# eezkni/UEGAN

Measured on AMD Instinct MI355X. Metric: train imgs/sec @512px bs=16 on 1/2/4/8 MI355X; infer ms/img, higher is better.
Workload: dtype bf16; 1 GPU; FiveK-shaped 512x512 batch=16/GPU, full G/D/VGG train step (trainer.py:77-119), conv_dim=32, seeded stand-in VGG19; global_batch=16, parallelism=dp1, pool_size=50, collective=none (1 rank), passes=batched (fused.py)

## Files before the change

include/uegan_hip.h:

```cpp
#ifndef UEGAN_HIP_H_
#define UEGAN_HIP_H_

#include <stddef.h>
#include <stdint.h>

#ifdef __cplusplus
extern "C" {
#endif

#define UEGAN_VERSION 105

enum { UEGAN_OK = 0, UEGAN_E_INVALID = -1, UEGAN_E_HIP = -2, UEGAN_E_UNSUPPORTED = -3 };
enum { UEGAN_F32 = 0, UEGAN_BF16 = 1 };
enum { UEGAN_PAD_ZERO = 0, UEGAN_PAD_REFLECT = 1 };
enum { UEGAN_ACT_NONE = 0, UEGAN_ACT_LRELU = 1, UEGAN_ACT_RELU = 2, UEGAN_ACT_TANH = 3,
       UEGAN_ACT_SIGMOID = 4,
       UEGAN_ACT_SWISH = 5, UEGAN_ACT_SELU = 6 };
enum { UEGAN_IMPL_AUTO = 0, UEGAN_IMPL_MFMA = 1, UEGAN_IMPL_DIRECT = 2, UEGAN_IMPL_MFMA_REGSTAGE = 3, UEGAN_IMPL_MFMA_GENERIC = 4 };

typedef void* uegan_stream_t;

int uegan_version(void);
const char* uegan_last_error(void);
int uegan_set_conv_impl(int impl);
enum {
  UEGAN_TUNE_SMALL_GRID = 0,
  UEGAN_TUNE_FOLD_MAX = 1,
  UEGAN_TUNE_HEADS_NO_CG = 2,
  UEGAN_TUNE_WIDE_MIN_GRID = 3,
  UEGAN_TUNE_TALL_MIN_GRID = 4,
  UEGAN_TUNE_TALL_RPW = 5,
  UEGAN_TUNE_TALL_REFLECT = 6,
  UEGAN_TUNE_FLAT_S2 = 7,
  UEGAN_TUNE_TOEP_HEADS = 8,
  UEGAN_TUNE_HEADS_MFMA = 9,
  UEGAN_TUNE_FWD_STATS = 10,
  UEGAN_TUNE_WGRAD_XCD = 11,
  UEGAN_TUNE_VGG_EPI = 12,
  UEGAN_TUNE_GAM_BWD = 13,
  UEGAN_TUNE_COUNT = 14
};
int uegan_set_tuning(int knob, int value, int* previous);
int uegan_selftest_mfma(void* scratch_4096_floats, uegan_stream_t stream);

typedef struct {
  char name[96];
  int64_t launches;
  double total_ms;
  double total_flops;
  double total_bytes;
} uegan_profile_entry;
int uegan_profile_begin(int max_records);
int uegan_profile_end(uegan_profile_entry* out, int max_entries, int* n_entries);

typedef struct {
  int32_t dtype;
  int32_t B, H, W;
  int32_t C1, C2;
  int32_t Ho, Wo, Cout;
  int32_t KH, KW, stride, pad;
  int32_t pad_mode;
  int32_t act;
  int32_t Cin_w, Cout_w;
// ... 181 lines not shown
int uegan_nima_dwconv3x3(const float* x_nhwc, const float* w_9c, const float* scale, const float* shift, float* y_nhwc, int B, int H, int W,
                         int C_pad, int stride, float lo, float hi, uegan_stream_t stream);
int uegan_nima_pwconv(const float* x_mk, const float* w_nk, const float* scale, const float* shift, const float* residual, float* y_mn,
                      int64_t M, int Cin_pad, int Cout_pad, float lo, float hi, uegan_stream_t stream);
int uegan_nima_head(const float* x_nhwc, const float* w, const float* bias, float* pooled, float* probs, float* mean, float* std, int B,
                    int HW, int C_pad, int C, int n_classes, uegan_stream_t stream);

int uegan_fill_zero(void* p, size_t bytes, uegan_stream_t stream);
int uegan_scalar_wsum(int n, const float* const* terms, const float* weights, float* total, float* scaled, uegan_stream_t stream);
int uegan_scalar_wsum_bwd(int n, const float* weights, const float* g, float* gout, uegan_stream_t stream);
int uegan_gather_scalars(int n, const float* const* src, float* out, uegan_stream_t stream);

size_t uegan_reduce_workspace_floats(int B, int HW, int C);
int uegan_instnorm_fwd(int dtype, const void* x, void* y, float* mean, float* rstd, float* tmp, int B, int HW, int C, float eps,
                       uegan_stream_t stream);
int uegan_instnorm_bwd(int dtype, const void* dy, const void* y, const float* rstd, void* dx, float* tmp, int B, int HW,
                       int C, uegan_stream_t stream);

size_t uegan_gam_bwd_ws_bytes(int dtype, int B, int HW, int C, int act);
int uegan_gam_bwd(int dtype, const void* g, const void* y, const void* x, const float* rstd, const void* w_ihwo, const void* add1,
                  const void* add2, int act, void* dz_enc, float* dw, int Cin_row, int Cin_w, int accumulate, void* workspace,
                  size_t workspace_bytes, int B, int HW, int C, uegan_stream_t stream);

int uegan_moments(int dtype, const void* x, float* mean, float* var, float* tmp, int B, int HW, int C, uegan_stream_t stream);
size_t uegan_moments_window_workspace_bytes(int B, int C);
int uegan_moments_window_acc(int dtype, const void* x, const void* x_lo, int B, int H, int W, int C, int y0, int y1, int x0, int x1, double* sum,
                             double* sumsq, void* tmp, uegan_stream_t stream);
int uegan_moments_finish(const double* sum, const double* sumsq, double count, float eps, float* mean, float* rstd, int n, uegan_stream_t stream);
int uegan_affine_act_fwd(int dtype, int act, const void* x, const float* scale, const float* shift, void* y, int B, int HW, int C,
                         uegan_stream_t stream);
int uegan_affine_act_bwd_sums(int dtype, int act, const void* gy, const void* x, const float* scale, const float* shift, float* sums,
                              float* tmp, int B, int HW, int C, uegan_stream_t stream);
int uegan_affine_act_bwd_apply(int dtype, int act, const void* gy, const void* x, const float* scale, const float* shift, const float* ca,
                               const float* cb, const float* cc, void* gx, int B, int HW, int C, uegan_stream_t stream);

size_t uegan_rahinge_workspace_floats(int nscales);
int uegan_rahinge_fwd(int nscales, const float* const* real, const float* const* fake, const int64_t* n,
                      int for_discriminator, float* loss, float* tmp, uegan_stream_t stream);
int uegan_rahinge_bwd(int nscales, const float* const* real, const float* const* fake, const int64_t* n,
                      int for_discriminator, const float* tmp, const float* gscale, float* const* greal,
                      float* const* gfake, uegan_stream_t stream);
size_t uegan_rahinge_heads_workspace_floats(int nscales);
int uegan_rahinge_heads_fwd(int dtype, int nscales, const void* const* maps, const int64_t* pix_per_image, int nb, int cp, int ngroups,
                            int npairs, const int32_t* pairs, int for_discriminator, float* loss, float* tmp, uegan_stream_t stream);
int uegan_rahinge_heads_bwd(int dtype, int nscales, const void* const* maps, const int64_t* pix_per_image, int nb, int cp, int ngroups,
                            int npairs, const int32_t* pairs, int for_discriminator, const float* tmp, const float* gscale,
// ... 83 lines not shown
```

uegan_amd/_lib.py:

```python
import ctypes as C
import os

_HERE = os.path.dirname(os.path.abspath(__file__))
LIB_PATH = os.path.join(_HERE, "libuegan_hip.so")
LIB_PATH_F16 = os.path.join(_HERE, "libuegan_hip_f16.so")

_lib = None
_lib_f16 = None
_use_f16 = False
_emulated = False

c_int, c_i64, c_f32, c_vp, c_sz = C.c_int, C.c_int64, C.c_float, C.c_void_p, C.c_size_t


class ConvDesc(C.Structure):
    _fields_ = [(n, C.c_int32) for n in ("dtype", "B", "H", "W", "C1", "C2", "Ho", "Wo", "Cout", "KH", "KW", "stride", "pad",
                                          "pad_mode", "act", "Cin_w", "Cout_w", "Cin_total", "scale_group")]


class ProfileEntry(C.Structure):
    _fields_ = [("name", C.c_char * 96), ("launches", c_i64), ("total_ms", C.c_double), ("total_flops", C.c_double),
                ("total_bytes", C.c_double)]


# ... 69 lines not shown
    "uegan_conv2d_wgrad_acc": (c_int, [C.POINTER(ConvDesc), c_vp, c_vp, c_vp, c_vp, c_vp, c_vp, c_vp, c_sz, c_int, c_vp]),
    "uegan_act_bwd": (c_int, [c_int, c_int, c_vp, c_vp, c_vp, c_i64, c_vp]),
    "uegan_act_bwd2": (c_int, [c_int, c_int, c_vp, c_vp, c_vp, c_vp, c_i64, c_vp]),
    "uegan_act_bwd3": (c_int, [c_int, c_int, c_vp, c_vp, c_vp, c_vp, c_vp, c_i64, c_vp]),
    "uegan_nchw_to_nhwc": (c_int, [c_int, c_vp, c_vp, c_int, c_int, c_int, c_int, c_int, C.POINTER(c_f32), C.POINTER(c_f32), c_vp]),
    "uegan_nhwc_to_nchw": (c_int, [c_int, c_vp, c_vp, c_int, c_int, c_int, c_int, c_int, C.POINTER(c_f32), c_vp]),
    "uegan_residual_clamp_fwd": (c_int, [c_int, c_vp, c_vp, c_vp, c_int, c_int, c_int, c_int, c_int, c_vp]),
    "uegan_residual_clamp_bwd": (c_int, [c_int, c_vp, c_vp, c_vp, c_vp, c_vp, c_int, c_int, c_int, c_int, c_int, c_vp]),
    "uegan_residual_clamp_bwd_act": (c_int, [c_int, c_int, c_vp, c_vp, c_vp, c_vp, c_vp, c_int, c_int, c_int, c_int, c_int, c_vp]),
    "uegan_mul_bwd_act": (c_int, [c_int, c_int, c_int, c_vp, c_vp, c_vp, c_vp, c_vp, c_i64, c_vp]),
    "uegan_mul_fwd": (c_int, [c_int, c_vp, c_vp, c_vp, c_i64, c_vp]),
    "uegan_mul_bwd": (c_int, [c_int, c_vp, c_vp, c_vp, c_vp, c_vp, c_i64, c_vp]),
    "uegan_upsample2x_fwd": (c_int, [c_int, c_vp, c_vp, c_int, c_int, c_int, c_int, c_vp]),
    "uegan_upsample2x_fwd_at": (c_int, [c_int, c_vp, c_vp, c_int, c_int, c_int, c_int, c_int, c_int, c_int, c_int, c_vp]),
    "uegan_upsample2x_bwd": (c_int, [c_int, c_vp, c_vp, c_int, c_int, c_int, c_int, c_vp]),
    "uegan_maxpool2x2_fwd": (c_int, [c_int, c_vp, c_vp, c_int, c_int, c_int, c_int, c_vp]),
    "uegan_maxpool2x2_bwd": (c_int, [c_int, c_vp, c_vp, c_vp, c_int, c_int, c_int, c_int, c_vp]),
    "uegan_maxpool2x2_bwd_act": (c_int, [c_int, c_int, c_vp, c_vp, c_vp, c_int, c_int, c_int, c_int, c_vp]),
    "uegan_reduce_workspace_floats": (c_sz, [c_int, c_int, c_int]),
    "uegan_instnorm_fwd": (c_int, [c_int, c_vp, c_vp, c_vp, c_vp, c_vp, c_int, c_int, c_int, c_f32, c_vp]),
    "uegan_instnorm_bwd": (c_int, [c_int, c_vp, c_vp, c_vp, c_vp, c_vp, c_int, c_int, c_int, c_vp]),
    "uegan_gam_bwd_ws_bytes": (c_sz, [c_int, c_int, c_int, c_int, c_int]),
    "uegan_gam_bwd": (c_int, [c_int, c_vp, c_vp, c_vp, c_vp, c_vp, c_vp, c_vp, c_int, c_vp, c_vp, c_int, c_int, c_int, c_vp, c_sz, c_int, c_int, c_int, c_vp]),
    "uegan_moments": (c_int, [c_int, c_vp, c_vp, c_vp, c_vp, c_int, c_int, c_int, c_vp]),
    "uegan_moments_window_workspace_bytes": (c_sz, [c_int, c_int]),
    "uegan_moments_window_acc": (c_int, [c_int, c_vp, c_vp, c_int, c_int, c_int, c_int, c_int, c_int, c_int, c_int, c_vp, c_vp, c_vp, c_vp]),
    "uegan_moments_finish": (c_int, [c_vp, c_vp, C.c_double, c_f32, c_vp, c_vp, c_int, c_vp]),
    "uegan_affine_act_fwd": (c_int, [c_int, c_int, c_vp, c_vp, c_vp, c_vp, c_int, c_int, c_int, c_vp]),
    "uegan_affine_act_bwd_sums": (c_int, [c_int, c_int, c_vp, c_vp, c_vp, c_vp, c_vp, c_vp, c_int, c_int, c_int, c_vp]),
    "uegan_affine_act_bwd_apply": (c_int, [c_int, c_int, c_vp, c_vp, c_vp, c_vp, c_vp, c_vp, c_vp, c_vp, c_int, c_int, c_int, c_vp]),
    "uegan_rals_fwd": (c_int, [c_int, C.POINTER(c_vp), C.POINTER(c_vp), C.POINTER(c_i64), c_int, c_vp, c_vp, c_vp]),
    "uegan_rals_bwd": (c_int, [c_int, C.POINTER(c_vp), C.POINTER(c_vp), C.POINTER(c_i64), c_int, c_vp, c_vp, C.POINTER(c_vp), C.POINTER(c_vp), c_vp]),
    "uegan_pred_loss_fwd": (c_int, [c_int, c_f32, c_int, C.POINTER(c_vp), C.POINTER(c_i64), c_vp, c_vp, c_vp]),
    "uegan_pred_loss_bwd": (c_int, [c_int, c_f32, c_int, C.POINTER(c_vp), C.POINTER(c_i64), c_vp, C.POINTER(c_vp), c_vp]),
    "uegan_rahinge_fwd": (c_int, [c_int, C.POINTER(c_vp), C.POINTER(c_vp), C.POINTER(c_i64), c_int, c_vp, c_vp, c_vp]),
    "uegan_rahinge_bwd": (c_int, [c_int, C.POINTER(c_vp), C.POINTER(c_vp), C.POINTER(c_i64), c_int, c_vp, c_vp, C.POINTER(c_vp),
                                  C.POINTER(c_vp), c_vp]),
    "uegan_rahinge_heads_workspace_floats": (c_sz, [c_int]),
    "uegan_rahinge_heads_fwd": (c_int, [c_int, c_int, C.POINTER(c_vp), C.POINTER(c_i64), c_int, c_int, c_int, c_int, C.POINTER(C.c_int32), c_int,
                                        c_vp, c_vp, c_vp]),
    "uegan_rahinge_heads_bwd": (c_int, [c_int, c_int, C.POINTER(c_vp), C.POINTER(c_i64), c_int, c_int, c_int, c_int, C.POINTER(C.c_int32), c_int,
                                        c_vp, c_vp, C.POINTER(c_vp), C.c_uint32, c_vp]),
    "uegan_msrec_scratch_floats": (c_sz, []),
    "uegan_msrec_fwd": (c_int, [c_vp, c_vp, c_vp, c_vp, c_int, c_int, c_int, c_int, c_int, c_int, c_vp]),
    "uegan_msrec_bwd": (c_int, [c_vp, c_vp, c_vp, c_vp, c_int, c_int, c_int, c_int, c_int, c_int, c_vp]),
    "uegan_msl1_scratch_floats": (c_sz, []),
# ... 135 lines not shown
```

uegan_amd/csrc/common.h:

```cpp
#pragma once
#include <hip/hip_runtime.h>
#include <stdint.h>
#include <stddef.h>

#include "../../include/uegan_hip.h"

#ifdef UEGAN_TOOLS_BUILD
#define UEGAN_ABL_BITS(x) (x)
#else
#define UEGAN_ABL_BITS(x) 0
#endif

namespace uegan {

extern int g_tuning[UEGAN_TUNE_COUNT];
extern int g_abl_stream, g_abl_wide;


typedef uint16_t bf16_t;

typedef float f32x4 __attribute__((ext_vector_type(4)));
typedef short s16x8 __attribute__((ext_vector_type(8)));
typedef uint32_t u32x4 __attribute__((ext_vector_type(4)));
typedef uint32_t u32x2 __attribute__((ext_vector_type(2)));
// ... 154 lines not shown
}

__device__ __forceinline__ void percep_scalars(float weight, const float* gscale, int B, int HW, int C, float& k, float& inv_n) {
  const float nel = (float)B * (float)HW * (float)C;
  k = 2.f * weight * (gscale ? *gscale : 1.f) / nel;
  inv_n = 1.f / (float)HW;
}
__device__ __forceinline__ void percep_consts(const float* st, const float* tot, size_t bc, size_t o, float k, float inv_n, float& mx, float& rx,
                                              float& my, float& ry, float& mg, float& mgx) {
  mx = st[o]; rx = st[bc + o]; my = st[2 * bc + o]; ry = st[3 * bc + o];
  mg = k * tot[o * 3 + 1] * inv_n;
  mgx = k * tot[o * 3 + 2] * inv_n;
}
__device__ __forceinline__ float percep_tap_grad(float x, float y, float mx, float rx, float my, float ry, float k, float mg, float mgx) {
  const float xh = (x - mx) * rx, yh = (y - my) * ry;
  return rx * (k * (xh - yh) - mg - xh * mgx);
}

__host__ __device__ __forceinline__ int reflect_idx(int i, int n) {
  i = i < 0 ? -i : i;
  return i >= n ? 2 * (n - 1) - i : i;
}

__device__ __forceinline__ float wave_sum(float v) {
#pragma unroll
  for (int o = 32; o > 0; o >>= 1) v += __shfl_xor(v, o, 64);
  return v;
}

__device__ __forceinline__ float block_sum(float v, float* red) {
  v = wave_sum(v);
  const int lane = threadIdx.x & 63, w = threadIdx.x >> 6;
  __syncthreads();
  if (lane == 0) red[w] = v;
  __syncthreads();
  const int nw = (blockDim.x + 63) >> 6;
  float s = 0.f;
  for (int i = 0; i < nw; ++i) s += red[i];
  return s;
}

template <int N>
__device__ __forceinline__ void wait_vmcnt() {
  __builtin_amdgcn_s_waitcnt((N & 15) | (7 << 4) | (15 << 8) | ((N >> 4) << 14));
}
__device__ __forceinline__ void raw_barrier() { __builtin_amdgcn_s_barrier(); }
// ... 22 lines not shown
```

uegan_amd/csrc/conv_internal.h:

```cpp
#pragma once
#include <hip/hip_runtime.h>

#include "../../include/uegan_hip.h"

namespace uegan {
bool heads_applicable(const uegan_conv_desc* d);
int heads_fwd(const uegan_conv_desc* d, const void* x, const void* w_ohwi, const float* bias, const float* scale, void* y, hipStream_t s);
bool heads_dgrad_applicable(const uegan_conv_desc* d);
int heads_dgrad(const uegan_conv_desc* d, const void* dz, const void* w_ihwo, const float* scale, void* dx, hipStream_t s);
int heads_wgrad_blocks(const uegan_conv_desc* d);
int heads_wgrad(const uegan_conv_desc* d, const void* x, const void* dz, float* ws, hipStream_t s);
void percep_tap_consts(int dtype, const float* tmp, int B, int HW, int C, const float** st, const float** tot);
int instnorm_bwd_sums(int dtype, const void* dy, const void* y, float* tmp, int B, int HW, int C, hipStream_t s, const float** tot);
int wgrad_reduce_1x1(const float* ws, float* dw, int nsplit, int N, int C, int Cin_w, int Cin_row, size_t pstride, int acc, hipStream_t s);
}
```

uegan_amd/csrc/elementwise.hip:

```cpp
#include "common.h"
#include "launch.h"

namespace uegan {

struct Affine4 {
  float a[4], b[4];
  int on;
};

template <typename T>
__global__ void nchw_to_nhwc_kernel(const float* x, T* y, int B, int C, int Cp, int HW, Affine4 af, int pair) {
  constexpr int EPC = DT<T>::EPC;
  const int nch = Cp / EPC;
  const size_t total = (size_t)B * HW * nch;
  for (size_t i = (size_t)blockIdx.x * blockDim.x + threadIdx.x; i < total; i += (size_t)gridDim.x * blockDim.x) {
    const int ch = (int)(i % nch);
    const size_t p = i / nch;
    const int b = (int)(p / HW);
    const size_t hw = p - (size_t)b * HW;
    float v[EPC];
#pragma unroll
    for (int e = 0; e < EPC; ++e) {
      const int c = ch * EPC + e;
      v[e] = 0.f;
// ... 67 lines not shown
    Vec<T, V>::ld(b + i, bv);
#pragma unroll
    for (int e = 0; e < V; ++e) av[e] *= bv[e];
    Vec<T, V>::st(y + i, av);
  }
}
template <typename T, int V>
__global__ void mul_bwd_kernel(const T* g, const T* a, const T* b, T* da, T* db, size_t n, int act_a, int act_b) {
  for (size_t i = ((size_t)blockIdx.x * blockDim.x + threadIdx.x) * V; i < n; i += (size_t)gridDim.x * blockDim.x * V) {
    float gv[V], av[V], bv[V];
    Vec<T, V>::ld(g + i, gv);
    Vec<T, V>::ld(a + i, av);
    Vec<T, V>::ld(b + i, bv);
#pragma unroll
    for (int e = 0; e < V; ++e) {
      const float t = gv[e];
      gv[e] = t * bv[e] * act_grad_from_out(av[e], act_a);
      bv[e] = t * av[e] * act_grad_from_out(bv[e], act_b);
    }
    Vec<T, V>::st(da + i, gv);
    Vec<T, V>::st(db + i, bv);
  }
}
__device__ __forceinline__ void bilinear_src(int o, int in_n, int out_n, int& i0, int& i1, float& l1) {
  const float scale = out_n > 1 ? (float)(in_n - 1) / (float)(out_n - 1) : 0.f;
  const float s = scale * (float)o;
  i0 = (int)s;
  i1 = i0 + (i0 < in_n - 1 ? 1 : 0);
  l1 = s - (float)i0;
}

template <typename T, int V>
__global__ void upsample2x_fwd_kernel(const T* x, T* y, int B, int H, int W, int C) {
  const int OH = 2 * H, OW = 2 * W, CV = C / V;
  const int row = blockIdx.y, b = row / OH, oy = row - b * OH;
  int y0, y1;
  float ly;
  bilinear_src(oy, H, OH, y0, y1, ly);
  const float hy = 1.f - ly;
  const T* r0 = x + ((size_t)b * H + y0) * W * C;
  const T* r1 = x + ((size_t)b * H + y1) * W * C;
  T* yo = y + (size_t)row * OW * C;
  for (int i = blockIdx.x * blockDim.x + threadIdx.x; i < OW * CV; i += gridDim.x * blockDim.x) {
    const int ox = i / CV, c = (i - ox * CV) * V;
    int x0, x1;
    float lx;
    bilinear_src(ox, W, OW, x0, x1, lx);
    float v00[V], v01[V], v10[V], v11[V];
    Vec<T, V>::ld(r0 + (size_t)x0 * C + c, v00);
    Vec<T, V>::ld(r0 + (size_t)x1 * C + c, v01);
    Vec<T, V>::ld(r1 + (size_t)x0 * C + c, v10);
    Vec<T, V>::ld(r1 + (size_t)x1 * C + c, v11);
    const float hx = 1.f - lx;
#pragma unroll
// ... 384 lines not shown
```

uegan_amd/csrc/runtime.hip:

```cpp
#include "conv_core.h"

#include <stdarg.h>

namespace uegan {

static thread_local char g_err[512] = "";

void set_error(const char* fmt, ...) {
  va_list ap;
  va_start(ap, fmt);
  vsnprintf(g_err, sizeof(g_err), fmt, ap);
  va_end(ap);
}

ConvImpl g_impl = {UEGAN_IMPL_AUTO, true, true, true, true, true};
int g_tuning[UEGAN_TUNE_COUNT] = {256, -1, 0, 192, 192, 0, 1, 1, 1, 1, 1, 1, 1, 1};
int g_abl_stream = 0, g_abl_wide = 0;
#ifdef UEGAN_TOOLS_BUILD
extern "C" int uegan_tools_set_ablation(int stream_wgrad_bits, int wide_variant) {
  g_abl_stream = stream_wgrad_bits;
  g_abl_wide = wide_variant;
  return UEGAN_OK;
}
#endif

bool g_prof_on = false;
std::vector<ProfRecord> g_prof_records;
std::vector<std::pair<hipEvent_t, hipEvent_t>> g_prof_pool;
size_t g_prof_used = 0;

__global__ void selftest_mfma_kernel(float* out) {
  const int lane = threadIdx.x & 63;
  f32x4 acc = {0.f, 0.f, 0.f, 0.f};
  const int ai = lane & 15, ak = lane >> 4;
  acc = mfma_f32(ai == ak ? 1.f : 0.f, 100.f * (lane >> 4) + (lane & 15), acc);
  for (int r = 0; r < 4; ++r) out[lane * 4 + r] = acc[r];
  __attribute__((aligned(16))) unsigned short av[8];
  __attribute__((aligned(16))) unsigned short bv[8];
  for (int e = 0; e < 8; ++e) {
// ... 105 lines not shown
```

uegan_amd/csrc/wgrad.hip:

```cpp
#include "conv_core.h"

namespace uegan {

struct WgradArgs {
  ConvGeom g;
  const void* in1;
  const void* in2;
  const void* dz;
  float* ws;
  int N, zC, ktot;
  int WS, WSlog, R;
  int nxb, nyb;
  int steps_total, steps_per_split;
};

constexpr int WG_BK = 128;

__device__ __forceinline__ void transpose_chunks(const u32x4 (&in)[4], u32x4 (&out)[4]) {
  out[0] = u32x4{in[0].x, in[1].x, in[2].x, in[3].x};
  out[1] = u32x4{in[0].y, in[1].y, in[2].y, in[3].y};
  out[2] = u32x4{in[0].z, in[1].z, in[2].z, in[3].z};
  out[3] = u32x4{in[0].w, in[1].w, in[2].w, in[3].w};
}
__device__ __forceinline__ void transpose_chunks(const u32x4 (&in)[8], u32x4 (&out)[8]) {
// ... 275 lines not shown
          if (sx < 0) continue;
          const size_t pix = ((size_t)b * g.IH + sy) * g.IW + sx;
          const float xv = (c < g.C1) ? DT<T>::ld(in1 + pix * g.C1 + c) : DT<T>::ld(in2 + pix * g.C2 + (c - g.C1));
          acc += xv * DT<T>::ld(dz + (((size_t)b * g.OH + oy) * g.OW + ox) * a.zC + n);
        }
      }
    float* o = dw + ((size_t)n * Cin_row + c) * (g.KH * g.KW) + tap;
    *o = acc * scale + (accum ? *o : 0.f);
  }
}

}

using namespace uegan;

int uegan::wgrad_reduce_1x1(const float* ws, float* dw, int nsplit, int N, int C, int Cin_w, int Cin_row, size_t pstride, int acc, hipStream_t s) {
  const size_t total = (size_t)N * C;
  hipLaunchKernelGGL(wgrad_reduce_kernel, dim3((unsigned)((total + 31) / 32)), dim3(256), 0, s, ws, dw, (float*)nullptr, (const float*)nullptr, nsplit, N, C,
                     Cin_w, 1, 1, pstride, acc, 0, Cin_row);
  UEGAN_CHECK_LAUNCH();
  return UEGAN_OK;
}

struct WgradPlan {
  WgradArgs a;
  WgradTrPlan tr;
  int nsplit, bn;
  dim3 grid;
  size_t ws_bytes;
};

static void wgrad_plan(const uegan_conv_desc* d, WgradPlan& p) {
  WgradArgs& a = p.a;
  a.g = fwd_geom(d);
  a.N = cout_w(d);
  a.zC = d->Cout;
  a.ktot = d->KH * d->KW * (d->C1 + d->C2);
  auto done = [&](int bn, int nsplit, dim3 grid) {
    p.bn = bn; p.nsplit = nsplit; p.grid = grid;
    p.ws_bytes = ((size_t)nsplit * ((size_t)a.N * a.ktot + a.N) + (size_t)BIAS_BLOCKS * d->Cout) * sizeof(float);
  };
  if (g_impl.impl != UEGAN_IMPL_DIRECT && wgtr_plan(d, a.g, p.tr)) return done(-1, p.tr.nsplit_eff, p.tr.grid);
  const int npix = d->dtype == UEGAN_BF16 ? 64 : 32;
  int ws = 1, wl = 0;
  while (ws < d->Wo && ws < npix) { ws <<= 1; ++wl; }
  a.WS = ws; a.WSlog = wl; a.R = npix / ws;
// ... 104 lines not shown
```

uegan_amd/models.py:

```python
import math


def _refuse_replica(m):
    if getattr(m, "_is_replica", False):
        raise RuntimeError("uegan_amd modules do not run as nn.DataParallel replicas (several device ids): use one process per GPU and "
                           "uegan_amd.trainer.Trainer -- see INTEGRATION.md")


import torch
import torch.nn as nn
import torch.nn.functional as F

from . import ops
from .ops.core import _sink_of
from . import variants


def _require(cond, what):
    if not cond:
        raise NotImplementedError("uegan_amd implements the reference's default configuration only: " + what)


class ReflectionPadTag(nn.Module):

# ... 252 lines not shown
        self.upsample4 = nn.Sequential(Interpolate(2, "bilinear", True), SNConv(cd * 2, cd * 1, 1, 1, 0, 1, True, use_sn))

        self.dec1 = ConvBlock(cd * 16, cd * 8, 3, 1, **kw)
        self.dec2 = ConvBlock(cd * 8, cd * 4, 3, 1, **kw)
        self.dec3 = ConvBlock(cd * 4, cd * 2, 3, 1, **kw)
        self.dec4 = ConvBlock(cd * 2, cd * 1, 3, 1, **kw)
        self.dec5 = nn.Sequential(SNConv(cd, cd, 3, 1, 0, 1, True, False), SNConv(cd, 3, 7, 1, 0, 1, True, False, act=ops.ACT_TANH),
                                  Identity())

        self.ga5 = GAM(cd * 16, cd * 16, reduction=8, bias=False, use_sn=use_sn, norm=True)
        self.ga4 = GAM(cd * 8, cd * 8, reduction=8, bias=False, use_sn=use_sn, norm=True)
        self.ga3 = GAM(cd * 4, cd * 4, reduction=8, bias=False, use_sn=use_sn, norm=True)
        self.ga2 = GAM(cd * 2, cd * 2, reduction=8, bias=False, use_sn=use_sn, norm=True)
        self.ga1 = GAM(cd * 1, cd * 1, reduction=8, bias=False, use_sn=use_sn, norm=True)
        self.dec5[1].main[1].cfg.premasked = True
        if not self.default_flags:
            return
        L = ops.ACT_LRELU
        for prod, cons in ((self.enc5, self.ga5), (self.dec1, self.upsample2[1]), (self.dec2, self.upsample3[1]), (self.dec3, self.upsample4[1])):
            prod.main[1].cfg.premasked = True
            (cons._cfg if isinstance(cons, GAM) else cons.main[1].cfg).in_act = L
        self.dec4.main[1].cfg.premasked = True

    @staticmethod
    def _up(block, x, ex=None, at=None):
        return block[0](block[1](x, ex=ex), at=at)

    @staticmethod
    def _check_input(x):
        if x.dim() != 4 or x.shape[1] != 3 or x.shape[2] % 16 or x.shape[3] % 16 or min(x.shape[2:]) < 32:
            raise RuntimeError("Generator expects [B,3,H,W] with H,W multiples of 16 and >= 32 (got %s)" % (tuple(x.shape),))

    def _precise(self):
        if not ops.precise():
            return False
        if not (self.default_flags and self.enc1.main[1].out_channels == 32):
            raise RuntimeError("uegan_amd.set_precise(True) covers the default generator (norm 'none', LeakyReLU, no spectral norm) at conv_dim 32; "
                               "call set_precise(False) for this network")
        return True

    def _check_tiled(self, what):
        if self.training or torch.is_grad_enabled():
            raise RuntimeError("Generator.%s is inference only: call it in eval mode under torch.no_grad()" % what)

    def forward(self, x, tile=None):
        _refuse_replica(self)
        self._check_input(x)
        if tile is not None:
# ... 157 lines not shown
```

uegan_amd/ops/__init__.py:

```python
from .. import _lib as L
from ..codecs import (JPEG_MAX_SIDE, JPEG_SUBSAMPLINGS, PNG_MAX_BAND, deflate_bands, jpeg_build_tables, jpeg_capacity,
                      jpeg_coeffs, jpeg_encode, jpeg_histogram, jpeg_qtables, jpeg_sizes, png_encode,
                      JpegDecodeError, JpegUnsupported, jpeg_decode, jpeg_decode_coeffs, jpeg_decode_into, jpeg_info)
from .conv import (ConvCfg, ConvExtras, PackedWeight, PackTable, SNCall, StatsHolder, _ConvFn, _desc, _sub_desc, conv2d,
                   raw_conv_dgrad, raw_conv_fwd, raw_conv_wgrad, refuse_stale_pack, specnorm_sigma, split_k)
from .core import (ACT_LRELU, ACT_NONE, ACT_RELU, ACT_TANH, IN_EPS, PAD_REFLECT, PAD_ZERO, SN_EPS, GradSink, _chk, _dt, _farr, _p,
                   _ptr_table, _sink_of, _stream, _weight_epoch, chunk_elems, cpad, fuse_epilogues, get_compute_dtype,
                   invalidate_weight_caches, lib, precise, set_compute_dtype, set_precise, workspace)
from .elementwise import (gam_bwd_ws_bytes, gam_hub, instnorm, instnorm_pair, maxpool2x2, moments_acc_new, moments_finish,
                          moments_window_acc, mul, raw_act_bwd, residual_clamp, residual_clamp_pair, upsample2x, zero_)
from .layout import copy_images, raw_to_nchw_grad, raw_to_nhwc, to_nchw, to_nhwc, to_nhwc_pair
from .loss import REC_KINDS, gather_scalars, loss_sum, multiscale_l1, multiscale_rec, perceptual_taps_loss, rahinge
from .optim import FusedAdamL2
```

uegan_amd/ops/elementwise.py:

```python
import torch

from .. import _lib as L
from .conv import StatsHolder, _wgrad_done, _wgrad_target, raw_conv_fwd, refuse_stale_pack
from .core import ACT_NONE, IN_EPS, _chk, _dt, _p, _sink_of, _stream, lib, workspace


class _Upsample2x(torch.autograd.Function):
    @staticmethod
    def forward(ctx, x):
        x = x.contiguous()
        B, H, W, Cc = x.shape
        y = torch.empty((B, 2 * H, 2 * W, Cc), dtype=x.dtype, device=x.device)
        _chk(x)
        L.check(lib().uegan_upsample2x_fwd(_dt(x), _p(x), _p(y), B, H, W, Cc, _stream()))
        return y

    @staticmethod
    def backward(ctx, g):
        g = g.contiguous()
        B, H2, W2, Cc = g.shape
        gx = torch.empty((B, H2 // 2, W2 // 2, Cc), dtype=g.dtype, device=g.device)
        L.check(lib().uegan_upsample2x_bwd(_dt(g), _p(g), _p(gx), B, H2 // 2, W2 // 2, Cc, _stream()))
        return gx

# ... 86 lines not shown
        x, y, stats, weight = ctx.saved_tensors
        cfg, d = ctx.cfg, ctx.d
        gy = gs[-1]
        adds = [g.contiguous() for g in gs[:-1] if g is not None]
        if gy is None or len(adds) > 2:
            raise RuntimeError("gam_hub backward: the attention output's gradient and at most two further gradients of x expected")
        refuse_stale_pack(cfg.packed, ctx.ihwo, ctx.pack_version,
                          "gam_hub backward: the module's weight was updated by an optimizer step after this forward; run backward() before step()")
        gy = gy.contiguous()
        _chk(gy, *adds)
        B, H, W, Cc = x.shape
        dz_enc = torch.empty_like(x)
        ws = workspace(ctx.wsb, x.device)
        sink, dw, _, acc = _wgrad_target(ctx.wsink, None, False, ctx.needs_input_grad[1], None, weight, cfg.cin_used, 0, x.device)
        L.check(lib().uegan_gam_bwd(_dt(x), _p(gy), _p(y), _p(x), _p(stats[1]), _p(ctx.ihwo), _p(adds[0]) if adds else None,
                                    _p(adds[1]) if len(adds) > 1 else None, ctx.x_act, _p(dz_enc), _p(dw), d.Cin_total, d.Cin_w, 1 if acc else 0,
                                    _p(ws), ctx.wsb, B, H * W, Cc, _stream()))
        dw, _ = _wgrad_done(sink, ctx.wsink, None, False, dw, None)
        return dz_enc, dw, None, None, None, None


def gam_hub(x, weight, cfg, x_act, n_x, wsb):
    return _GamHub.apply(x, weight, cfg, x_act, n_x, wsb)


class _Mul(torch.autograd.Function):
    @staticmethod
    def forward(ctx, a, b, act_a, act_b, given=None):
        ctx.acts = (act_a, act_b)
        a, b = a.contiguous(), b.contiguous()
        _chk(a, b)
        if given is not None:
            y = given.view_as(given)
        else:
            y = torch.empty_like(a)
            L.check(lib().uegan_mul_fwd(_dt(a), _p(a), _p(b), _p(y), a.numel(), _stream()))
        ctx.save_for_backward(a, b)
        return y

    @staticmethod
    def backward(ctx, g):
        a, b = ctx.saved_tensors
        g = g.contiguous()
        da, db = torch.empty_like(a), torch.empty_like(b)
        L.check(lib().uegan_mul_bwd_act(_dt(a), ctx.acts[0], ctx.acts[1], _p(g), _p(a), _p(b), _p(da), _p(db), a.numel(), _stream()))
        return da, db, None, None, None
# ... 151 lines not shown
```

Baseline: 512.5 imgs/sec.

## Fuse bilinear upsample backward with 1x1 conv dgrad/wgrad in decoder up-projections

Adds a dedicated HIP kernel for the backward pass of the decoder's 1x1 conv followed by a 2x bilinear upsample. A single streaming, ring-buffered pass computes the downsampled gradient in LDS, then uses MFMA for weight and bias gradients (with per-block partials reduced afterwards) and for the input gradient with the LeakyReLU mask applied. This removes the separate upsample-backward kernel, the intermediate gradient tensor round-trip through memory, and the separate dgrad/wgrad launches. In exchange it adds a large special-cased kernel limited to two channel shapes and bf16, plus a workspace-based split reduction.

```diff
diff --git a/include/uegan_hip.h b/include/uegan_hip.h
--- a/include/uegan_hip.h
+++ b/include/uegan_hip.h
@@ -38,7 +38,8 @@
   UEGAN_TUNE_WGRAD_XCD = 11,
   UEGAN_TUNE_VGG_EPI = 12,
   UEGAN_TUNE_GAM_BWD = 13,
-  UEGAN_TUNE_COUNT = 14
+  UEGAN_TUNE_UPPROJ_BWD = 14,
+  UEGAN_TUNE_COUNT = 15
 };
 int uegan_set_tuning(int knob, int value, int* previous);
 int uegan_selftest_mfma(void* scratch_4096_floats, uegan_stream_t stream);
@@ -266,6 +267,10 @@
                   const void* add2, int act, void* dz_enc, float* dw, int Cin_row, int Cin_w, int accumulate, void* workspace,
                   size_t workspace_bytes, int B, int HW, int C, uegan_stream_t stream);
 
+size_t uegan_upproj_bwd_ws_bytes(int dtype, int B, int H, int W, int Cin, int Cout, int in_act);
+int uegan_upproj_bwd(int dtype, const void* g_up, const void* x, const void* w_ihwo, int in_act, void* dx, float* dw, float* dbias, int accumulate,
+                     void* workspace, size_t workspace_bytes, int B, int H, int W, int Cin, int Cout, uegan_stream_t stream);
+
 int uegan_moments(int dtype, const void* x, float* mean, float* var, float* tmp, int B, int HW, int C, uegan_stream_t stream);
 size_t uegan_moments_window_workspace_bytes(int B, int C);
 int uegan_moments_window_acc(int dtype, const void* x, const void* x_lo, int B, int H, int W, int C, int y0, int y1, int x0, int x1, double* sum,
diff --git a/uegan_amd/_lib.py b/uegan_amd/_lib.py
--- a/uegan_amd/_lib.py
+++ b/uegan_amd/_lib.py
@@ -115,6 +115,8 @@
     "uegan_instnorm_bwd": (c_int, [c_int, c_vp, c_vp, c_vp, c_vp, c_vp, c_int, c_int, c_int, c_vp]),
     "uegan_gam_bwd_ws_bytes": (c_sz, [c_int, c_int, c_int, c_int, c_int]),
     "uegan_gam_bwd": (c_int, [c_int, c_vp, c_vp, c_vp, c_vp, c_vp, c_vp, c_vp, c_int, c_vp, c_vp, c_int, c_int, c_int, c_vp, c_sz, c_int, c_int, c_int, c_vp]),
+    "uegan_upproj_bwd_ws_bytes": (c_sz, [c_int, c_int, c_int, c_int, c_int, c_int, c_int]),
+    "uegan_upproj_bwd": (c_int, [c_int, c_vp, c_vp, c_vp, c_int, c_vp, c_vp, c_vp, c_int, c_vp, c_sz, c_int, c_int, c_int, c_int, c_int, c_vp]),
     "uegan_moments": (c_int, [c_int, c_vp, c_vp, c_vp, c_vp, c_int, c_int, c_int, c_vp]),
     "uegan_moments_window_workspace_bytes": (c_sz, [c_int, c_int]),
     "uegan_moments_window_acc": (c_int, [c_int, c_vp, c_vp, c_int, c_int, c_int, c_int, c_int, c_int, c_int, c_int, c_vp, c_vp, c_vp, c_vp]),
diff --git a/uegan_amd/csrc/common.h b/uegan_amd/csrc/common.h
--- a/uegan_amd/csrc/common.h
+++ b/uegan_amd/csrc/common.h
@@ -200,6 +200,14 @@
   return i >= n ? 2 * (n - 1) - i : i;
 }
 
+__device__ __forceinline__ void bilinear_src(int o, int in_n, int out_n, int& i0, int& i1, float& l1) {
+  const float scale = out_n > 1 ? (float)(in_n - 1) / (float)(out_n - 1) : 0.f;
+  const float s = scale * (float)o;
+  i0 = (int)s;
+  i1 = i0 + (i0 < in_n - 1 ? 1 : 0);
+  l1 = s - (float)i0;
+}
+
 __device__ __forceinline__ float wave_sum(float v) {
 #pragma unroll
   for (int o = 32; o > 0; o >>= 1) v += __shfl_xor(v, o, 64);
diff --git a/uegan_amd/csrc/conv_internal.h b/uegan_amd/csrc/conv_internal.h
--- a/uegan_amd/csrc/conv_internal.h
+++ b/uegan_amd/csrc/conv_internal.h
@@ -13,4 +13,5 @@
 void percep_tap_consts(int dtype, const float* tmp, int B, int HW, int C, const float** st, const float** tot);
 int instnorm_bwd_sums(int dtype, const void* dy, const void* y, float* tmp, int B, int HW, int C, hipStream_t s, const float** tot);
 int wgrad_reduce_1x1(const float* ws, float* dw, int nsplit, int N, int C, int Cin_w, int Cin_row, size_t pstride, int acc, hipStream_t s);
+int wgrad_reduce_1x1_bias(const float* ws, float* dw, float* dbias, int nsplit, int N, int C, size_t pstride, int acc, int accb, hipStream_t s);
 }
diff --git a/uegan_amd/csrc/elementwise.hip b/uegan_amd/csrc/elementwise.hip
--- a/uegan_amd/csrc/elementwise.hip
+++ b/uegan_amd/csrc/elementwise.hip
@@ -113,14 +113,6 @@
     Vec<T, V>::st(db + i, bv);
   }
 }
-__device__ __forceinline__ void bilinear_src(int o, int in_n, int out_n, int& i0, int& i1, float& l1) {
-  const float scale = out_n > 1 ? (float)(in_n - 1) / (float)(out_n - 1) : 0.f;
-  const float s = scale * (float)o;
-  i0 = (int)s;
-  i1 = i0 + (i0 < in_n - 1 ? 1 : 0);
-  l1 = s - (float)i0;
-}
-
 template <typename T, int V>
 __global__ void upsample2x_fwd_kernel(const T* x, T* y, int B, int H, int W, int C) {
   const int OH = 2 * H, OW = 2 * W, CV = C / V;
diff --git a/uegan_amd/csrc/runtime.hip b/uegan_amd/csrc/runtime.hip
--- a/uegan_amd/csrc/runtime.hip
+++ b/uegan_amd/csrc/runtime.hip
@@ -14,7 +14,7 @@
 }
 
 ConvImpl g_impl = {UEGAN_IMPL_AUTO, true, true, true, true, true};
-int g_tuning[UEGAN_TUNE_COUNT] = {256, -1, 0, 192, 192, 0, 1, 1, 1, 1, 1, 1, 1, 1};
+int g_tuning[UEGAN_TUNE_COUNT] = {256, -1, 0, 192, 192, 0, 1, 1, 1, 1, 1, 1, 1, 1, 1};
 int g_abl_stream = 0, g_abl_wide = 0;
 #ifdef UEGAN_TOOLS_BUILD
 extern "C" int uegan_tools_set_ablation(int stream_wgrad_bits, int wide_variant) {
diff --git a/uegan_amd/csrc/upproj_bwd.hip b/uegan_amd/csrc/upproj_bwd.hip
--- /dev/null
+++ b/uegan_amd/csrc/upproj_bwd.hip
@@ -0,0 +1,343 @@
+#include "conv_core.h"
+
+namespace uegan {
+
+struct UpProjArgs {
+  const bf16_t *g, *x, *w;
+  bf16_t* dx;
+  float* ws;
+  int H, W, act;
+  int strips, tiles_total, tiles_per_block;
+};
+
+__device__ __forceinline__ void upproj_weights(int i, int n, float (&w)[6]) {
+#pragma unroll
+  for (int k = 0; k < 6; ++k) {
+    const int o = 2 * i - 2 + k;
+    float v = 0.f;
+    if (i < n && o >= 0 && o < 2 * n) {
+      int i0, i1;
+      float l;
+      bilinear_src(o, n, 2 * n, i0, i1, l);
+      if (i0 == i) v += 1.f - l;
+      if (i1 == i) v += l;
+    }
+    w[k] = v;
+  }
+}
+
+template <int CIN, int COUT>
+__global__ void __launch_bounds__(256, 2) upproj_bwd_kernel(UpProjArgs a) {
+  constexpr int CHO = COUT / 8, CHI = CIN / 8;
+  constexpr int TP = 256 / CHO;
+  constexpr int RW = 2 * TP + 4;
+  constexpr int RBG = 2 * COUT;
+  constexpr int RING = RW * RBG;
+  constexpr int RBX = 2 * CIN;
+  constexpr int DRB = 4 * CIN + 16;
+  constexpr int HALO = 4 * CHO;
+  constexpr int KD = COUT / 32;
+  constexpr int WPP = 4 / (TP / 16);
+  constexpr int NCO = COUT / 16, NCI = CIN / 16;
+  constexpr int WPC = 4 / NCO, TM = NCI / WPC;
+  constexpr int KW = TP / 32;
+  static_assert(CIN == 2 * COUT && (COUT == 32 || COUT == 64), "upsample4 (64 -> 32) and upsample3 (128 -> 64)");
+  __shared__ __attribute__((aligned(16))) unsigned char lds[6 * RING + TP * RBG + TP * RBX + TP * DRB];
+  unsigned char* const ring = lds;
+  unsigned char* const zs = lds + 6 * RING;
+  unsigned char* const xs = zs + TP * RBG;
+  unsigned char* const ds = xs + TP * RBX;
+  const int tid = threadIdx.x, lane = tid & 63;
+  const int wave = __builtin_amdgcn_readfirstlane(tid >> 6);
+  const int cq = tid % CHO, prow = tid / CHO;
+  const int OH = 2 * a.H, OW = 2 * a.W;
+
+  const int g4 = lane >> 4, sj = (lane & 15) >> 2, seg = lane & 3;
+  const int pk = sj + 4 * (g4 & 1) + 16 * (g4 >> 1);
+  auto tr_addr = [&](int rb, int ch) { return pk * rb + ((((ch >> 3) ^ wgtr_swz(rb, pk))) << 4) + ((ch >> 2) & 1) * 8; };
+  const int co_t = wave / WPC, ci_t0 = (wave % WPC) * TM;
+  const int zaddr = tr_addr(RBG, co_t * 16 + 4 * seg);
+  int xaddr[TM];
+#pragma unroll
+  for (int m = 0; m < TM; ++m) xaddr[m] = tr_addr(RBX, (ci_t0 + m) * 16 + 4 * seg);
+  const int ptile = wave / WPP, mt0 = (wave % WPP) * 4;
+  u32x4 wf[4][KD];
+#pragma unroll
+  for (int mt = 0; mt < 4; ++mt)
+#pragma unroll
+    for (int ks = 0; ks < KD; ++ks) wf[mt][ks] = *reinterpret_cast<const u32x4*>(a.w + ((mt0 + mt) * 16 + (lane & 15)) * COUT + ks * 32 + 8 * g4);
+  const unsigned int one2 = pack_bf16x2(1.f, 1.f);
+  const u32x4 ones = u32x4{one2, one2, one2, one2};
+
+  constexpr int FOLD = 8;
+  const f32x4 zf = f32x4{0.f, 0.f, 0.f, 0.f};
+  f32x4 accw[TM], totw[TM], accb = zf, totb = zf;
+#pragma unroll
+  for (int m = 0; m < TM; ++m) accw[m] = totw[m] = zf;
+
+  const int t_begin = blockIdx.x * a.tiles_per_block;
+  int t_end = t_begin + a.tiles_per_block;
+  if (t_end > a.tiles_total) t_end = a.tiles_total;
+
+  const u32x4 zero4 = u32x4{0u, 0u, 0u, 0u};
+  auto load_g = [&](int b, int oy, int ix0, int idx) -> u32x4 {
+    int col = 2 * ix0 - 2 + idx / CHO;
+    col = col < 0 ? 0 : (col > OW - 1 ? OW - 1 : col);
+    oy = oy < 0 ? 0 : (oy > OH - 1 ? OH - 1 : oy);
+    return *reinterpret_cast<const u32x4*>(a.g + (((size_t)b * OH + oy) * OW + col) * COUT + (idx % CHO) * 8);
+  };
+  auto ring_at = [&](int oy, int idx) { return ring + ((oy + 6) % 6) * RING + idx * 16; };
+  struct Operands { u32x4 g[2][2], gh, x[2]; };
+  auto load_x = [&](int b, int iy, int ix0, Operands& o) {
+#pragma unroll
+    for (int it = 0; it < 2; ++it) {
+      const int idx = it * 256 + tid;
+      const bool valid = ix0 + idx / CHI < a.W;
+      o.x[it] = *reinterpret_cast<const u32x4*>(a.x + (((size_t)b * a.H + iy) * a.W + ix0) * CIN + (size_t)(valid ? idx : idx % CHI) * 8);
+    }
+  };
+  auto load_step = [&](int b, int iy, int ix0, Operands& o) {
+#pragma unroll
+    for (int r = 0; r < 2; ++r)
+#pragma unroll
+      for (int it = 0; it < 2; ++it) o.g[r][it] = load_g(b, 2 * iy + 2 + r, ix0, it * 256 + tid);
+    o.gh = load_g(b, 2 * iy + 2 + (tid / HALO & 1), ix0, 512 + tid % HALO);
+    load_x(b, iy, ix0, o);
+  };
+  auto split = [&](int t, int& b, int& s, int& iy) {
+    b = t / (a.strips * a.H);
+    const int rem = t - b * (a.strips * a.H);
+    s = rem / a.H;
+    iy = rem - s * a.H;
+  };
+
+  Operands cur;
+  bool stepped = false;
+  float wxv[6];
+  int s_have = -1;
+  int b = 0, s = 0, iy = 0;
+  if (t_begin < t_end) {
+    split(t_begin, b, s, iy);
+    load_x(b, iy, s * TP, cur);
+  }
+  u32x4 pend[2];
+  int pend_b = -1, pend_iy = 0, pend_ix0 = 0;
+  auto flush = [&]() {
+    if (pend_b < 0) return;
+#pragma unroll
+    for (int it = 0; it < 2; ++it) {
+      const int idx = it * 256 + tid;
+      if (pend_ix0 + idx / CHI < a.W)
+        *reinterpret_cast<u32x4*>(a.dx + (((size_t)pend_b * a.H + pend_iy) * a.W + pend_ix0) * CIN + (size_t)idx * 8) = pend[it];
+    }
+  };
+  wait_vmcnt<0>();
+  for (int t = t_begin; t < t_end; ++t) {
+    const int ix0 = s * TP;
+    if (s != s_have) {
+      s_have = s;
+      upproj_weights(ix0 + prow, a.W, wxv);
+    }
+    float wyv[6];
+    upproj_weights(iy, a.H, wyv);
+    if (stepped) {
+#pragma unroll
+      for (int r = 0; r < 2; ++r)
+#pragma unroll
+        for (int it = 0; it < 2; ++it) *reinterpret_cast<u32x4*>(ring_at(2 * iy + 2 + r, it * 256 + tid)) = cur.g[r][it];
+      if (tid < 2 * HALO) *reinterpret_cast<u32x4*>(ring_at(2 * iy + 2 + tid / HALO, 512 + tid % HALO)) = cur.gh;
+    } else {
+      for (int k = 0; k < 6; ++k) {
+        const int oy = 2 * iy - 2 + k;
+        for (int idx = tid; idx < RW * CHO; idx += 256) *reinterpret_cast<u32x4*>(ring_at(oy, idx)) = load_g(b, oy, ix0, idx);
+      }
+    }
+    u32x4 xk[2];
+#pragma unroll
+    for (int it = 0; it < 2; ++it) {
+      const int idx = it * 256 + tid, p = idx / CHI, c = idx % CHI;
+      xk[it] = ix0 + p < a.W ? cur.x[it] : zero4;
+      *reinterpret_cast<u32x4*>(xs + p * RBX + ((c ^ wgtr_swz(RBX, p)) << 4)) = xk[it];
+    }
+    flush();
+    stepped = t + 1 < t_end && iy + 1 < a.H;
+    int b2 = b, s2 = s, iy2 = iy + 1;
+    if (iy2 == a.H) {
+      iy2 = 0;
+      if (++s2 == a.strips) { s2 = 0; ++b2; }
+    }
+    if (stepped) load_step(b, iy2, ix0, cur);
+    else if (t + 1 < t_end) load_x(b2, iy2, s2 * TP, cur);
+    __syncthreads();
+    {
+      float acc[8];
+#pragma unroll
+      for (int e = 0; e < 8; ++e) acc[e] = 0.f;
+#pragma unroll
+      for (int ky = 0; ky < 6; ++ky) {
+        const float wy = wyv[ky];
+        if (wy == 0.f) continue;
+        const unsigned char* grow = ring_at(2 * iy - 2 + ky, 2 * prow * CHO + cq);
+#pragma unroll
+        for (int kx = 0; kx < 6; ++kx) {
+          const float wx = wxv[kx];
+          if (wx == 0.f) continue;
+          const u32x4 gq = *reinterpret_cast<const u32x4*>(grow + kx * RBG);
+          float gv[8];
+#pragma unroll
+          for (int d = 0; d < 4; ++d) { gv[2 * d] = half_lo_to_f32(gq[d]); gv[2 * d + 1] = half_hi_to_f32(gq[d]); }
+#pragma unroll
+          for (int e = 0; e < 8; ++e) acc[e] += wy * wx * gv[e];
+        }
+      }
+      u32x4 z;
+#pragma unroll
+      for (int d = 0; d < 4; ++d) z[d] = pack_bf16x2(acc[2 * d], acc[2 * d + 1]);
+      *reinterpret_cast<u32x4*>(zs + prow * RBG + ((cq ^ wgtr_swz(RBG, prow)) << 4)) = z;
+    }
+    __syncthreads();
+    {
+      u32x4 af[KW];
+#pragma unroll
+      for (int ks = 0; ks < KW; ++ks) {
+        const u32x2 zl = lds_read_tr16(zs + ks * 32 * RBG + zaddr), zh = lds_read_tr16(zs + ks * 32 * RBG + zaddr + 8 * RBG);
+        af[ks] = u32x4{zl.x, zl.y, zh.x, zh.y};
+      }
+#pragma unroll
+      for (int m = 0; m < TM; ++m) {
+        f32x4 part[KW];
+#pragma unroll
+        for (int ks = 0; ks < KW; ++ks) {
+          const u32x2 xl = lds_read_tr16(xs + ks * 32 * RBX + xaddr[m]), xh = lds_read_tr16(xs + ks * 32 * RBX + xaddr[m] + 8 * RBX);
+          part[ks] = mfma_bf16(af[ks], u32x4{xl.x, xl.y, xh.x, xh.y}, f32x4{0.f, 0.f, 0.f, 0.f});
+        }
+        if constexpr (KW == 2) accw[m] += part[0] + part[1];
+        else accw[m] += part[0];
+      }
+      if (ci_t0 == 0) {
+        f32x4 part[KW];
+#pragma unroll
+        for (int ks = 0; ks < KW; ++ks) part[ks] = mfma_bf16(af[ks], ones, f32x4{0.f, 0.f, 0.f, 0.f});
+        if constexpr (KW == 2) accb += part[0] + part[1];
+        else accb += part[0];
+      }
+    }
+    if (((t - t_begin) & (FOLD - 1)) == FOLD - 1) {
+#pragma unroll
+      for (int m = 0; m < TM; ++m) { totw[m] += accw[m]; accw[m] = zf; }
+      totb += accb; accb = zf;
+    }
+    {
+      const int px = ptile * 16 + (lane & 15);
+      f32x4 accd[4];
+#pragma unroll
+      for (int mt = 0; mt < 4; ++mt) accd[mt] = f32x4{0.f, 0.f, 0.f, 0.f};
+#pragma unroll
+      for (int ks = 0; ks < KD; ++ks) {
+        const u32x4 bf = *reinterpret_cast<const u32x4*>(zs + px * RBG + (((ks * 4 + g4) ^ wgtr_swz(RBG, px)) << 4));
+#pragma unroll
+        for (int mt = 0; mt < 4; ++mt) accd[mt] = mfma_bf16(wf[mt][ks], bf, accd[mt]);
+      }
+#pragma unroll
+      for (int mt = 0; mt < 4; ++mt) *reinterpret_cast<f32x4*>(ds + px * DRB + ((mt0 + mt) * 16 + 4 * g4) * 4) = accd[mt];
+    }
+    __syncthreads();
+#pragma unroll
+    for (int it = 0; it < 2; ++it) {
+      const int idx = it * 256 + tid, p = idx / CHI, c = idx % CHI;
+      const f32x4 d0 = *reinterpret_cast<const f32x4*>(ds + p * DRB + c * 32), d1 = *reinterpret_cast<const f32x4*>(ds + p * DRB + c * 32 + 16);
+      const float v[8] = {d0.x, d0.y, d0.z, d0.w, d1.x, d1.y, d1.z, d1.w};
+      u32x4 o;
+#pragma unroll
+      for (int d = 0; d < 4; ++d) {
+        const float m0 = act_grad_from_out(half_lo_to_f32(xk[it][d]), a.act), m1 = act_grad_from_out(half_hi_to_f32(xk[it][d]), a.act);
+        if constexpr (COUT == 32) {
+          const unsigned int vr = pack_bf16x2(v[2 * d], v[2 * d + 1]);
+          o[d] = a.act == UEGAN_ACT_NONE ? vr : pack_bf16x2(half_lo_to_f32(vr) * m0, half_hi_to_f32(vr) * m1);
+        } else {
+          o[d] = pack_bf16x2(v[2 * d] * m0, v[2 * d + 1] * m1);
+        }
+      }
+      pend[it] = o;
+    }
+    pend_b = b; pend_iy = iy; pend_ix0 = ix0;
+    b = b2; s = s2; iy = iy2;
+  }
+  flush();
+  float* ws = a.ws + (size_t)blockIdx.x * (COUT * CIN + COUT);
+#pragma unroll
+  for (int m = 0; m < TM; ++m)
+#pragma unroll
+    for (int r = 0; r < 4; ++r) ws[(co_t * 16 + g4 * 4 + r) * CIN + (ci_t0 + m) * 16 + (lane & 15)] = totw[m][r] + accw[m][r];
+  if (ci_t0 == 0 && (lane & 15) == 0) {
+#pragma unroll
+    for (int r = 0; r < 4; ++r) ws[COUT * CIN + co_t * 16 + g4 * 4 + r] = totb[r] + accb[r];
+  }
+}
+
+static int upproj_blocks() {
+#if defined(UEGAN_EMU)
+  return 8;
+#else
+  return 512;
+#endif
+}
+
+struct UpProjPlan {
+  int strips, tiles_total, blocks;
+};
+
+static bool upproj_plan(int dtype, int B, int H, int W, int Cin, int Cout, int act, UpProjPlan& p) {
+  if (dtype != UEGAN_BF16 || !((Cin == 64 && Cout == 32) || (Cin == 128 && Cout == 64)) || B <= 0 || H <= 0 || W <= 0) return false;
+  if (act != UEGAN_ACT_NONE && act != UEGAN_ACT_LRELU) return false;
+  if (g_impl.impl == UEGAN_IMPL_DIRECT || !g_impl.glds || (Cout == 32 ? (!g_impl.stream || H < 16 || W < 32) : !g_impl.patch)) return false;
+  const int tp = 2048 / Cout;
+  p.strips = (W + tp - 1) / tp;
+  if ((long long)B * p.strips * H > (1 << 30) || (long long)H * W > (1 << 28)) return false;
+  p.tiles_total = B * p.strips * H;
+  p.blocks = p.tiles_total < upproj_blocks() ? p.tiles_total : upproj_blocks();
+  return true;
+}
+static void upproj_grid(const UpProjPlan& p, int cap, int& blocks, int& per_block) {
+  if (cap > p.blocks) cap = p.blocks;
+  if (cap < 1) cap = 1;
+  per_block = (p.tiles_total + cap - 1) / cap;
+  blocks = (p.tiles_total + per_block - 1) / per_block;
+}
+
+}
+
+using namespace uegan;
+
+extern "C" size_t uegan_upproj_bwd_ws_bytes(int dtype, int B, int H, int W, int Cin, int Cout, int in_act) {
+  const int knob = g_tuning[UEGAN_TUNE_UPPROJ_BWD];
+  UpProjPlan p;
+  if (knob == 0 || !upproj_plan(dtype, B, H, W, Cin, Cout, in_act, p)) return 0;
+  int blocks, per_block;
+  upproj_grid(p, knob >= 2 ? knob : p.blocks, blocks, per_block);
+  return (size_t)blocks * ((size_t)Cout * Cin + Cout) * sizeof(float);
+}
+
+extern "C" int uegan_upproj_bwd(int dtype, const void* g_up, const void* x, const void* w_ihwo, int in_act, void* dx, float* dw, float* dbias,
+                                int accumulate, void* workspace, size_t workspace_bytes, int B, int H, int W, int Cin, int Cout,
+                                uegan_stream_t stream) {
+  UpProjPlan p;
+  UEGAN_CHECK_ARG(upproj_plan(dtype, B, H, W, Cin, Cout, in_act, p),
+                  "uegan_upproj_bwd: 16-bit storage, 64 -> 32 or 128 -> 64 channels, activation none or LeakyReLU (ask uegan_upproj_bwd_ws_bytes first)");
+  UEGAN_CHECK_ARG(g_up && x && w_ihwo && dx && dw && dbias && workspace, "uegan_upproj_bwd: null argument");
+  UEGAN_CHECK_ARG(accumulate >= 0 && accumulate <= 3, "uegan_upproj_bwd: accumulate is a bit mask: 1 = dw, 2 = dbias");
+  const size_t per = (size_t)Cout * Cin + Cout, room = workspace_bytes / sizeof(float) / per;
+  UEGAN_CHECK_ARG(room >= 1, "uegan_upproj_bwd: workspace too small (uegan_upproj_bwd_ws_bytes)");
+  int blocks, per_block;
+  upproj_grid(p, room < (size_t)p.blocks ? (int)room : p.blocks, blocks, per_block);
+  hipStream_t s = (hipStream_t)stream;
+  UpProjArgs a;
+  a.g = static_cast<const bf16_t*>(g_up); a.x = static_cast<const bf16_t*>(x); a.w = static_cast<const bf16_t*>(w_ihwo);
+  a.dx = static_cast<bf16_t*>(dx); a.ws = static_cast<float*>(workspace);
+  a.H = H; a.W = W; a.act = in_act;
+  a.strips = p.strips; a.tiles_total = p.tiles_total; a.tiles_per_block = per_block;
+  if (Cout == 32) hipLaunchKernelGGL((upproj_bwd_kernel<64, 32>), dim3(blocks), dim3(256), 0, s, a);
+  else hipLaunchKernelGGL((upproj_bwd_kernel<128, 64>), dim3(blocks), dim3(256), 0, s, a);
+  UEGAN_CHECK_LAUNCH();
+  return wgrad_reduce_1x1_bias(a.ws, dw, dbias, blocks, Cout, Cin, per, accumulate & 1, (accumulate >> 1) & 1, s);
+}
diff --git a/uegan_amd/csrc/wgrad.hip b/uegan_amd/csrc/wgrad.hip
--- a/uegan_amd/csrc/wgrad.hip
+++ b/uegan_amd/csrc/wgrad.hip
@@ -321,6 +321,14 @@
   return UEGAN_OK;
 }
 
+int uegan::wgrad_reduce_1x1_bias(const float* ws, float* dw, float* dbias, int nsplit, int N, int C, size_t pstride, int acc, int accb, hipStream_t s) {
+  const size_t total = (size_t)N * C + N;
+  hipLaunchKernelGGL(wgrad_reduce_kernel, dim3((unsigned)((total + 31) / 32)), dim3(256), 0, s, ws, dw, dbias, (const float*)nullptr, nsplit, N, C, C, 1, 1,
+                     pstride, acc, accb, C);
+  UEGAN_CHECK_LAUNCH();
+  return UEGAN_OK;
+}
+
 struct WgradPlan {
   WgradArgs a;
   WgradTrPlan tr;
diff --git a/uegan_amd/models.py b/uegan_amd/models.py
--- a/uegan_amd/models.py
+++ b/uegan_amd/models.py
@@ -298,8 +298,14 @@
             (cons._cfg if isinstance(cons, GAM) else cons.main[1].cfg).in_act = L
         self.dec4.main[1].cfg.premasked = True
 
-    @staticmethod
-    def _up(block, x, ex=None, at=None):
+    def _up(self, block, x, ex=None, at=None):
+        conv = block[1].main[1]
+        if self.default_flags and ex is None and at is None and torch.is_grad_enabled() and not ops.precise() \
+                and isinstance(conv, Conv2d) and conv.kernel_size == 1 and conv.bias is not None and conv.cfg.act == ops.ACT_NONE:
+            B, H, W, _ = x.shape
+            wsb = ops.upproj_bwd_ws_bytes(x.dtype, B, H, W, conv.in_channels, conv.out_channels, conv.cfg.in_act)
+            if wsb:
+                return ops.upproj_hub(x, conv.weight, conv.bias, conv.cfg, wsb)
         return block[0](block[1](x, ex=ex), at=at)
 
     @staticmethod
diff --git a/uegan_amd/ops/__init__.py b/uegan_amd/ops/__init__.py
--- a/uegan_amd/ops/__init__.py
+++ b/uegan_amd/ops/__init__.py
@@ -8,7 +8,8 @@
                    _ptr_table, _sink_of, _stream, _weight_epoch, chunk_elems, cpad, fuse_epilogues, get_compute_dtype,
                    invalidate_weight_caches, lib, precise, set_compute_dtype, set_precise, workspace)
 from .elementwise import (gam_bwd_ws_bytes, gam_hub, instnorm, instnorm_pair, maxpool2x2, moments_acc_new, moments_finish,
-                          moments_window_acc, mul, raw_act_bwd, residual_clamp, residual_clamp_pair, upsample2x, zero_)
+                          moments_window_acc, mul, raw_act_bwd, residual_clamp, residual_clamp_pair, upproj_bwd_ws_bytes, upproj_hub, upsample2x,
+                          zero_)
 from .layout import copy_images, raw_to_nchw_grad, raw_to_nhwc, to_nchw, to_nhwc, to_nhwc_pair
 from .loss import REC_KINDS, gather_scalars, loss_sum, multiscale_l1, multiscale_rec, perceptual_taps_loss, rahinge
 from .optim import FusedAdamL2
diff --git a/uegan_amd/ops/elementwise.py b/uegan_amd/ops/elementwise.py
--- a/uegan_amd/ops/elementwise.py
+++ b/uegan_amd/ops/elementwise.py
@@ -132,6 +132,48 @@
 
 def gam_hub(x, weight, cfg, x_act, n_x, wsb):
     return _GamHub.apply(x, weight, cfg, x_act, n_x, wsb)
+
+
+def upproj_bwd_ws_bytes(dtype, B, H, W, Cin, Cout, in_act):
+    if dtype == torch.float32:
+        return 0
+    return lib().uegan_upproj_bwd_ws_bytes(1, B, H, W, Cin, Cout, in_act)
+
+
+class _UpProjHub(torch.autograd.Function):
+
+    @staticmethod
+    def forward(ctx, x, weight, bias, cfg, wsb):
+        x = x.contiguous()
+        v, d, ihwo = raw_conv_fwd(x, None, weight, bias, cfg)
+        B, H, W, Cc = v.shape
+        u = torch.empty((B, 2 * H, 2 * W, Cc), dtype=v.dtype, device=v.device)
+        L.check(lib().uegan_upsample2x_fwd(_dt(v), _p(v), _p(u), B, H, W, Cc, _stream()))
+        ctx.cfg, ctx.d, ctx.ihwo, ctx.pack_version, ctx.wsb = cfg, d, ihwo, cfg.packed.version, wsb
+        ctx.wsink, ctx.bsink = _sink_of(weight), _sink_of(bias)
+        ctx.save_for_backward(x, weight)
+        return u
+
+    @staticmethod
+    def backward(ctx, g):
+        x, weight = ctx.saved_tensors
+        cfg, d = ctx.cfg, ctx.d
+        refuse_stale_pack(cfg.packed, ctx.ihwo, ctx.pack_version,
+                          "upproj_hub backward: the layer's weight was updated by an optimizer step after this forward; run backward() before step()")
+        g = g.contiguous()
+        _chk(g)
+        B, H, W, Cin = x.shape
+        dx = torch.empty_like(x)
+        ws = workspace(ctx.wsb, x.device)
+        sink, dw, db, acc = _wgrad_target(ctx.wsink, ctx.bsink, True, ctx.needs_input_grad[1], None, weight, None, d.Cout_w, x.device)
+        L.check(lib().uegan_upproj_bwd(_dt(x), _p(g), _p(x), _p(ctx.ihwo), cfg.in_act, _p(dx), _p(dw), _p(db), acc, _p(ws), ctx.wsb,
+                                       B, H, W, Cin, d.Cout, _stream()))
+        dw, db = _wgrad_done(sink, ctx.wsink, ctx.bsink, True, dw, db)
+        return dx, dw, db, None, None
+
+
+def upproj_hub(x, weight, bias, cfg, wsb):
+    return _UpProjHub.apply(x, weight, bias, cfg, wsb)
 
 
 class _Mul(torch.autograd.Function):
```

After: 513.8 imgs/sec (median of 4 runs). Within noise of the previous version (+0.2%).
